# cerbos/cerbos

Measured on AMD Instinct MI355X. Metric: CheckResources decisions/sec at batch=1M; p50 per-decision us, higher is better.
Workload: dtype u32 ids + f64 attributes (CEL int64/uint64/double)

## Files before the change

cerbos_amd/csrc/cbh_check_flat.h:

```cpp
#pragma once
#include "cbh_check_wave.h"

#define CBH_FLAT_MAX_DEPTH 16
#if defined(CBH_FLAT_WAVES_OVERRIDE)
#define CBH_FLAT_WAVES CBH_FLAT_WAVES_OVERRIDE
#elif !defined(CBH_HOSTSIM)
#define CBH_FLAT_WAVES 4u
#else
#define CBH_FLAT_WAVES 1u
#endif
#define CBH_FLAT_THREADS (CBH_FLAT_WAVES * CBH_BLOCK)

__device__ __forceinline__ u64 wave_or64(u64 v, u32 wave, u32 lane) {
  __shared__ unsigned long long acc[CBH_FLAT_WAVES];
#ifndef CBH_HOSTSIM
  if (lane == 0) __hip_atomic_store(&acc[wave], 0ull, __ATOMIC_RELAXED, __HIP_MEMORY_SCOPE_WORKGROUP);
  (void)wave_ballot(true);
  if (v) (void)__hip_atomic_fetch_or(&acc[wave], (unsigned long long)v, __ATOMIC_RELAXED, __HIP_MEMORY_SCOPE_WORKGROUP);
  (void)wave_ballot(true);
  const u64 r = __hip_atomic_load(&acc[wave], __ATOMIC_RELAXED, __HIP_MEMORY_SCOPE_WORKGROUP);
#else
  if (lane == 0) acc[wave] = 0;
  (void)wave_ballot(true);
  if (v) atomicOr(&acc[wave], (unsigned long long)v);
  (void)wave_ballot(true);
  const u64 r = acc[wave];
#endif
  (void)wave_ballot(true);
  return r;
}

#define CBH_FLAT_LDS_STRINGS 4096u
struct u32x4u { u32 x, y, z, w; };
__device__ __forceinline__ u32x4u load_u32x4(const CBH_G u32* p) {
#ifndef CBH_HOSTSIM
  typedef u32 v4 __attribute__((ext_vector_type(4), aligned(4)));
  const v4 v = *(const CBH_G v4*)p;
  return u32x4u{v.x, v.y, v.z, v.w};
#else
  return u32x4u{p[0], p[1], p[2], p[3]};
#endif
}
template <int NDW> struct StagedRec { u32 w[NDW]; };
template <int NDW>
__device__ __forceinline__ StagedRec<NDW> stage_rec(const CBH_G u32* base, u32 idx, bool wanted) {
  StagedRec<NDW> r;
#pragma unroll
  for (int k = 0; k < NDW; ++k) r.w[k] = 0;
  if (wanted) {
    const CBH_G u32* p = base + (size_t)idx * NDW;
#pragma unroll
    for (int k = 0; k < NDW; k += 4) { const u32x4u v = load_u32x4(p + k); r.w[k] = v.x; r.w[k + 1] = v.y; r.w[k + 2] = v.z; r.w[k + 3] = v.w; }
  }
  return r;
}
template <typename R, int NDW>
__device__ __forceinline__ R staged_take(const StagedRec<NDW>& s, u32 lane) {
  static_assert(sizeof(R) == NDW * 4, "record size");
  u32 w[NDW];
#pragma unroll
  for (int k = 0; k < NDW; ++k) w[k] = wave_readlane(s.w[k], lane);
  R r;
  __builtin_memcpy(&r, w, sizeof(R));
  return r;
}
__device__ __forceinline__ u32 ctz64(u64 v) { return (u32)__builtin_ctzll(v); }
__device__ __forceinline__ u32 nz01(u32 v) {
#ifndef CBH_HOSTSIM
  u32 r;
  asm("v_min_u32 %0, 1, %1" : "=v"(r) : "v"(v));
  return r;
#else
  return v ? 1u : 0u;
#endif
}

template <typename T>
__device__ __forceinline__ void store_nt(CBH_G T* p, T v) {
#ifndef CBH_HOSTSIM
  __builtin_nontemporal_store(v, p);
#else
  *p = v;
#endif
}

struct __attribute__((aligned(64))) TblDrx { u32 rm_lo, rm_hi, flags, cond, name, p0, p1, p2; LeafRec leaf; };

struct FlatCol { u32 t, lo, hi; };
template <bool PT = false>
__device__ __forceinline__ FlatCol flat_col(const Ctx& c, u32 col, u32 req) {
  FlatCol v;
  v.t = cached_tag<PT>(c, col, req);
  v.lo = c.cc[col * CBH_BLOCK + c.tid];
  v.hi = c.cc[(c.n_cached + col) * CBH_BLOCK + c.tid];
  return v;
}
template <bool LISTS = true, bool PT = false>
__device__ __forceinline__ u32 flat_leaf(const Ctx& c, const LeafRec& lr, u32 req, u32 pid) {
  const u32 a = lr.w >> 8;
  const u32 ka = (a >> 8) & 0xFu, op = a & 0xFFu;
  const bool want_eq = op == OP_EQ;
  switch (lr.pad) {
    case 1: {
      const FlatCol x = flat_col<PT>(c, lr.a0, req);
      const bool err = x.t >= CBH_T_ABSENT;
      const bool eq = x.t == lr.ctag && x.lo == lr.clo;
      return err ? 2u : (u32)(eq == want_eq);
    }
    case 2: {
      const FlatCol x = flat_col<PT>(c, lr.a0, req);
      const bool err = x.t >= CBH_T_ABSENT;
      const bool dbl = x.t == CBH_T_DOUBLE, othernum = x.t == CBH_T_INT || x.t == CBH_T_UINT;
      const double p = as_f64((u64)x.lo | ((u64)x.hi << 32)), q = as_f64((u64)lr.clo | ((u64)lr.chi << 32));
      const bool ordering = op != OP_EQ && op != OP_NE;
      const bool cmp = (op == OP_EQ) ? p == q : (op == OP_NE) ? p != q : (op == OP_LT) ? p < q : (op == OP_LE) ? p <= q
                     : (op == OP_GT) ? p > q : p >= q;
      const bool slow = !err && othernum;
      const bool overload = !dbl && !othernum && ordering;
      const u32 r = dbl ? (u32)cmp : (u32)(op == OP_NE);
      return (err || overload) ? 2u : slow ? 4u : r;
    }
    case 3: {
      const FlatCol x = flat_col<PT>(c, lr.a0, req), y = flat_col<PT>(c, lr.a1, req);
      const bool err = x.t >= CBH_T_ABSENT || y.t >= CBH_T_ABSENT;
      const bool same = x.t == y.t;
      const bool scalar = x.t < CBH_T_LIST || x.t == CBH_T_TIMESTAMP || x.t == CBH_T_DURATION;
      const bool xnum = x.t == CBH_T_INT || x.t == CBH_T_UINT || x.t == CBH_T_DOUBLE, ynum = y.t == CBH_T_INT || y.t == CBH_T_UINT || y.t == CBH_T_DOUBLE;
      const bool bits_eq = x.lo == y.lo && x.hi == y.hi;
      const bool dbl_eq = as_f64((u64)x.lo | ((u64)x.hi << 32)) == as_f64((u64)y.lo | ((u64)y.hi << 32));
      const bool eq = same && (x.t == CBH_T_DOUBLE ? dbl_eq : bits_eq);
      const bool slow = !err && ((same && !scalar) || (!same && xnum && ynum));
      return err ? 2u : slow ? 4u : (u32)(eq == want_eq);
    }
    case 4: {
      const FlatCol x = flat_col<PT>(c, ka == 3 ? lr.a0 : lr.a1, req);
      const bool err = x.t >= CBH_T_ABSENT;
      const bool eq = x.t == CBH_T_STRING && x.lo == pid;
      return err ? 2u : (u32)(eq == want_eq);
    }
    case 6: {
      const FlatCol x = flat_col<PT>(c, lr.a0, req);
      const bool err = x.t >= CBH_T_ABSENT;
      const bool found = x.t == CBH_T_STRING && (x.lo == lr.ctag || x.lo == lr.clo || x.lo == lr.chi);
      return err ? 2u : (u32)found;
    }
    case 7:
    case 8: {
      if (!LISTS) return 4u;
      const FlatCol h = flat_col<PT>(c, lr.a1, req);
      u32 nt = CBH_T_STRING, nlo = lr.clo;
      bool err = h.t >= CBH_T_ABSENT;
      if (lr.pad == 8u) {
        if (ka == 4u) nlo = pid;
        else { const FlatCol x = flat_col<PT>(c, lr.a0, req); nt = x.t; nlo = x.lo; err = err || x.t >= CBH_T_ABSENT; }
      }
      const bool is_map = h.t == CBH_T_MAP, cont = h.t == CBH_T_LIST || is_map;
      const u32 sel = h.hi >> 30, off = h.hi & 0x3FFFFFFFu, len = cont ? h.lo : 0u, stride = is_map ? 2u : 1u;
      const bool slow = !err && (nt != CBH_T_STRING || (cont && (sel != CBH_HEAP_BATCH || len > 64u)));
      const u32 n = (err || slow) ? 0u : len;
      bool found = false;
      for (u32 i = 0; wave_ballot(i < n) != 0; i += 4u) {
        u32 tg[4]; u32 vl[4];
#pragma unroll
        for (u32 q = 0; q < 4; ++q) {
          const u32 at = off + stride * (i + q < n ? i + q : (n ? n - 1u : 0u));
          tg[q] = n ? (u32)c.b.heap_tag[at] : 0u; vl[q] = n ? (u32)c.b.heap_val[at] : 0u;
        }
#pragma unroll
        for (u32 q = 0; q < 4; ++q) found = found || (i + q < n && tg[q] == CBH_T_STRING && vl[q] == nlo);
      }
      return (err || (!slow && !cont)) ? 2u : slow ? 4u : (u32)found;
    }
    default: return 4u;
  }
}

template <bool LISTS = true, bool PT = false>
__device__ __forceinline__ u32 flat_tree(const Ctx& c, const LeafRec& desc, u32 req, u32 pid) {
  const u32 opw[4] = {desc.w, desc.a0, desc.ret, desc.ctag};
  bool live = true, last = false;
  u32 saved = 0, acc = 0, depth = 0, leaf = desc.a1, err = 0, slow = 0;
  for (u32 k = 0; k < 32; ++k) {
    const u32 ws = k >> 3, word = ws == 0u ? opw[0] : ws == 1u ? opw[1] : ws == 2u ? opw[2] : opw[3];
    const u32 op = (word >> (4u * (k & 7u))) & 15u;
    if (op == 0) break;
    if (op == 1) {
      const LeafRec lr = uload_rec<LeafRec>(c.t.code, leaf++);
      const u32 lv = flat_leaf<LISTS, PT>(c, lr, req, pid);
      last = live && (lv & 1u) != 0;
      err |= live ? (lv & 2u) : 0u;
      slow |= live ? (lv & 4u) : 0u;
    } else if (op < 5) {
      const u32 bit = 1u << depth;
      saved = live ? (saved | bit) : (saved & ~bit);
      acc = (op == 2) ? (acc | bit) : (acc & ~bit);
      ++depth;
    } else if (op < 8) {
      const u32 bit = 1u << (depth - 1u);
      const bool decides = live && ((op == 5) ? !last : last);
      acc = decides ? ((op == 5) ? (acc & ~bit) : (acc | bit)) : acc;
      live = live && !decides;
    } else {
      --depth;
      const u32 bit = 1u << depth;
      live = (saved & bit) != 0;
      last = ((acc & bit) != 0) != (op == 10);
    }
  }
  return slow ? 4u : ((u32)last | err);
}

__device__ __forceinline__ u32 wave_max_bits(u32 v, bool in, u32 nbits) {
  u32 best = 0;
  for (u32 k = nbits; k-- > 0;) {
    const bool bit = ((v >> k) & 1u) != 0;
    if (wave_ballot(in && bit) != 0) { in = in && bit; best |= 1u << k; }
  }
  return best;
}

#define CBH_LV_ROWS 16u
__device__ __forceinline__ u32 lv_code(const CBH_L u8* lvtab, u32 tid, u32 leaf) {
  return ((u32)lvtab[(leaf >> 2) * CBH_BLOCK + tid] >> ((leaf & 3u) * 2u)) & 3u;
}
__device__ __forceinline__ u32 lv_of_code(u32 code) { return code == 3u ? 4u : code; }
struct __attribute__((aligned(64))) Leaf4x4 { u32 w[16]; };
template <bool PT>
__device__ __forceinline__ void leaf_col(const Ctx& c, u32 w, u32 req, u32& curcol, FlatCol& x) {
  const u32 col = (w >> 16) & 0xFFu;
  if (col != curcol) { x = flat_col<PT>(c, col, req); curcol = col; }
}
template <bool PT>
__device__ __forceinline__ u32 leaf_block_codes(const Ctx& c, const Leaf4x4& b, u32 req, u32 pid, u32& curcol, FlatCol& x) {
  const u32 cls = b.w[0] & 15u;
  u32 acc = 0;
  if (cls == 1u) {
#pragma unroll
    for (u32 q = 0; q < 4; ++q) {
      const u32 w = b.w[4 * q];
      leaf_col<PT>(c, w, req, curcol, x);
      const bool ne = ((w >> 4) & 0xFFu) != OP_EQ;
      const bool eq = x.t == b.w[4 * q + 1] && x.lo == b.w[4 * q + 2];
      acc |= (x.t >= CBH_T_ABSENT ? 2u : (u32)(eq != ne)) << (2u * q);
    }
  } else if (cls == 2u) {
#pragma unroll
    for (u32 q = 0; q < 4; ++q) {
      const u32 w = b.w[4 * q], op = (w >> 4) & 0xFFu;
      leaf_col<PT>(c, w, req, curcol, x);
      const bool a_lt = op == OP_LT || op == OP_LE || op == OP_NE, a_eq = op == OP_EQ || op == OP_LE || op == OP_GE,
                 a_gt = op == OP_GT || op == OP_GE || op == OP_NE, a_un = op == OP_NE;
      const double p = as_f64((u64)x.lo | ((u64)x.hi << 32)), k = as_f64((u64)b.w[4 * q + 1] | ((u64)b.w[4 * q + 2] << 32));
      const bool lt = p < k, eq = p == k, gt = p > k;
      const bool cmp = (a_lt && lt) || (a_eq && eq) || (a_gt && gt) || (a_un && !(lt || eq || gt));
      const bool dbl = x.t == CBH_T_DOUBLE, othernum = x.t == CBH_T_INT || x.t == CBH_T_UINT;
      const bool ordering = op != OP_EQ && op != OP_NE;
      const u32 r = dbl ? (u32)cmp : (u32)(op == OP_NE);
// ... 207 lines not shown
    act_off = 4u * req;
  } else {
#define RQ(f) b.req_u32[(size_t)(f) * NR + req]
  pid = RQ(CBH_RQ_PRINCIPAL_ID); kind = RQ(CBH_RQ_KIND); r_scope = RQ(CBH_RQ_R_SCOPE); r_ver = RQ(CBH_RQ_R_VERSION);
  role_off = RQ(CBH_RQ_ROLE_OFF); act_off = RQ(CBH_RQ_ACT_OFF);
  role_cnt = valid ? RQ(CBH_RQ_ROLE_CNT) : 0; act_cnt = valid ? RQ(CBH_RQ_ACT_CNT) : 0;
#undef RQ
  if constexpr (AGROUP) {
    act_total = act_cnt;
    const u32 g4 = 4u * ag.group, left = act_cnt > g4 ? act_cnt - g4 : 0u;
    act_cnt = left < 4u ? left : 4u; act_off += g4;
  }
  if constexpr (!AGROUP) {
  spec = b.n_tuples >= 4u;
  spec_ix = (4u * req + 4u <= b.n_tuples) ? 4u * req : 0u;
  sp = load_u32x4(spec ? b.tuple_action + spec_ix : b.req_u32);
  }
  const u32 cls_i = threadIdx.x < t.K ? threadIdx.x : kmax;
  cls_a0 = (t.K ? t.action_class : (const CBH_G u8*)b.req_u32)[cls_i]; cls_r0 = (t.K ? t.role_class : (const CBH_G u8*)b.req_u32)[cls_i];
  }
  CcTags cct;
  if constexpr (COMPACT) { for (u32 g = 0; g < CBH_CACHE_COLS / 4; ++g) cct.w[g] = 0; } else cct = cc_load_tags(c, b, NR, w0, wd);
  const bool ptags = COMPACT || (c.flags & CBH_FI_PACKED_TAGS) != 0;
  const u32 all = CROSS ? ((1u << act_cnt) - 1u) & ~x_done : (1u << act_cnt) - 1u;
  const u32 max_depth = t.max_depth < CBH_FLAT_MAX_DEPTH ? t.max_depth : CBH_FLAT_MAX_DEPTH;
  const bool chain8 = t.n_scopes <= 256u;
  const u32 chain_dwords = chain8 ? max_depth * (CBH_BLOCK / 4u) : max_depth * CBH_BLOCK;
  CBH_L u32* chain_si = (CBH_L u32*)cbh_dyn_lds + CBH_FLAT_WAVES * CBH_CC_DWORDS(c.n_cached, ptags) + wave * chain_dwords;
  CBH_L u8* chain_si8 = (CBH_L u8*)chain_si;
  const bool cls_in_lds = t.K <= CBH_FLAT_LDS_STRINGS;
  CBH_L u8* cls_lds = (CBH_L u8*)((CBH_L u32*)cbh_dyn_lds + CBH_FLAT_WAVES * (CBH_CC_DWORDS(c.n_cached, ptags) + chain_dwords));
  u32 aid[4] = {0, 0, 0, 0}, rid[4] = {0, 0, 0, 0};
  if constexpr (!COMPACT) {
#pragma unroll
  for (u32 k = 0; k < 4; ++k) rid[k] = b.roles[k < role_cnt ? role_off + k : 0u];
  const bool spec_hit = spec && act_cnt == 4u && act_off == spec_ix;
  aid[0] = sp.x; aid[1] = sp.y; aid[2] = sp.z; aid[3] = sp.w;
  if (!spec_hit) {
#pragma unroll
    for (u32 k = 0; k < 4; ++k) aid[k] = b.tuple_action[k < act_cnt ? act_off + k : 0u];
  }
  if (cls_in_lds) {
    if (threadIdx.x < t.K) { cls_lds[threadIdx.x] = (u8)cls_a0; cls_lds[t.K + threadIdx.x] = (u8)cls_r0; }
    for (u32 i = threadIdx.x + CBH_FLAT_THREADS; i < t.K; i += CBH_FLAT_THREADS) { cls_lds[i] = t.action_class[i]; cls_lds[t.K + i] = t.role_class[i]; }
  }
  }
  CBH_L u64* segm = (CBH_L u64*)(cls_lds + (cls_in_lds ? ((2u * t.K + 15u) & ~15u) : 0u)) + wave * (CBH_SEG_LDS_BYTES / 8u);
  CBH_L u8* seg_rec = (CBH_L u8*)(segm + 64);
  CBH_L u64* seg_desc = segm + 64 + 16;
  CBH_L u8* lvtab = (CBH_L u8*)(segm + 64 + 16 + 64);
  CBH_L u32* ep_lds = (CBH_L u32*)(cls_lds + (cls_in_lds ? ((2u * t.K + 15u) & ~15u) : 0u) + (MODE == 2 ? CBH_FLAT_WAVES * CBH_SEG_LDS_BYTES : 0u)) + wave * max_depth * 2u * CBH_BLOCK;
  const bool want_ep = EP && (flags & CBH_F_WANT_EFFECTIVE_POLICIES) != 0 && o.eff_pol != nullptr;
  if (EP) { for (u32 d = 0; d < 2u * max_depth; ++d) ep_lds[d * CBH_BLOCK + c.tid] = 0; }
  if constexpr (CROSS) cc_fill_cross(c, b, NR, x_prow, x_rrow, x.side); else if constexpr (!COMPACT) cc_fill(c, b, NR, w0, wd, cct);
  const bool lenient = (flags & CBH_F_LENIENT_SCOPE_SEARCH) != 0;
  u32 first_own;
  if constexpr (COMPACT) first_own = c_first; else first_own = chain_first(t, r_scope, FLAG_RES, lenient);
  const u32 first = (AGROUP && ag.group != 0u && act_cnt == 0u) ? CBH_NONE : first_own;
  if constexpr (COMPACT) {
  } else if (cls_in_lds) {
    __syncthreads();
#pragma unroll
    for (u32 k = 0; k < 4; ++k) {
      const u32 ca = cls_lds[aid[k] < t.K ? aid[k] : kmax], cr = cls_lds[t.K + (rid[k] < t.K ? rid[k] : kmax)];
      ac[k] = (k < act_cnt && aid[k] < t.K && ca < 31u) ? ca : 31u;
      rc[k] = (k < role_cnt && rid[k] < t.K && cr < 31u) ? cr : 31u;
    }
  } else {
#pragma unroll
    for (u32 k = 0; k < 4; ++k) {
      const u32 ca = t.action_class[aid[k] < t.K ? aid[k] : kmax], cr = t.role_class[rid[k] < t.K ? rid[k] : kmax];
      ac[k] = (k < act_cnt && aid[k] < t.K && ca < 31u) ? ca : 31u;
      rc[k] = (k < role_cnt && rid[k] < t.K && cr < 31u) ? cr : 31u;
    }
  }
  u32 lane_ac = 0, lane_rc = 0;
  u32 walks = 0;
#pragma unroll
  for (u32 k = 0; k < 4; ++k) {
    if (k < act_cnt) lane_ac |= 1u << ac[k];
    if (k < role_cnt) { lane_rc |= 1u << rc[k]; walks |= all << (4 * k); }
  }
  const u64 wave_cls = wave_or64((u64)lane_ac | ((u64)lane_rc << 32), wave, c.tid);
  const u32 wave_ac = (u32)wave_cls, wave_rc = (u32)(wave_cls >> 32);
  FLAT_DBG(const u64 cyc1 = __builtin_readcyclecounter();)

  Lane L; L.req = req; L.edr = 0; L.status = 0; L.edr_err = false; L.pid = pid;

  u32 S = walks;
  u32 has_allow = 0, allow = 0, deny = 0, err = 0, unsup = 0;
  u32 dp0 = 0, dp1 = 0, dp2 = 0, dp3 = 0;
  const u32 scope_bits = t.n_scopes > 1 ? 32u - (u32)__builtin_clz(t.n_scopes - 1u) : 0u;

  auto leafish = [&](u32 ref, u32 how, const LeafRec& lr, bool active) -> u32 {
    u32 lv = 4u;
    FLAT_DBG(const u64 e0 = __builtin_readcyclecounter(); ++dbg_evals;)
    if (how == 1u) lv = flat_leaf<WITH_CALL || CROSS, COMPACT>(c, lr, req, pid);
    else if (how == 2u) lv = flat_tree<WITH_CALL || CROSS, COMPACT>(c, lr, req, pid);
    FLAT_DBG(cyc_eval += (__builtin_readcyclecounter() - e0) * (u64)(wave_ballot(lv != 77u) != 0);)
    const bool slow = active && lv == 4u;
    if (WITH_CALL) {
      if (wave_ballot(slow) != 0) {
        const u32 r = eval_ref<false>(c.ka_mem, lds_of(c), req, 0, false, ref, slow);
        if (slow) lv = ((r & 0xFFu) == 1u ? 1u : 0u) | (((r >> 8) & CBH_ST_CEL_ERROR) ? 2u : 0u) | (((r >> 8) & CBH_ST_UNSUPPORTED) ? 8u : 0u);
      }
    } else if (slow) lv = 8u;
    return active ? lv : 0u;
  };

  u32 memo_r0 = CBH_NONE, memo_r1 = CBH_NONE, memo_r2 = CBH_NONE, memo_r3 = CBH_NONE, memo_n = 0;
  u32 memo_lv = 0;
  auto leafish_memo = [&](u32 ref, u32 how, auto&& leaf, bool active) -> u32 {
    if constexpr (WITH_CALL || !MEMO) return leafish(ref, how, leaf(), active);
    else {
      const u32 j = ref == memo_r0 ? 0u : ref == memo_r1 ? 1u : ref == memo_r2 ? 2u : ref == memo_r3 ? 3u : 4u;
      if (j < 4u) return active ? ((memo_lv >> (4u * j)) & 15u) : 0u;
      const u32 lv = leafish(ref, how, leaf(), true);
      if (memo_n < 4u) {
        memo_r0 = memo_n == 0u ? ref : memo_r0; memo_r1 = memo_n == 1u ? ref : memo_r1; memo_r2 = memo_n == 2u ? ref : memo_r2; memo_r3 = memo_n == 3u ? ref : memo_r3;
        memo_lv |= lv << (4u * memo_n);
        ++memo_n;
      }
      return active ? lv : 0u;
    }
  };

  u32 cur = first, mydepth = 0;
  bool exists = false;
  const bool pooled = MODE == 2 && (t.seg_info & CBH_MSEG_POOLED) != 0;
  u32 blocks_done = 0;
  FLAT_DBG(const u64 cyc2 = cyc1 + (__builtin_readcyclecounter() - cyc1) * (u64)(wave_ballot(first != 0xFFFFFFFEu) != 0);)
  for (;;) {
    const bool active = cur != CBH_NONE && (S != 0 || !exists);
    if (wave_ballot(active) == 0) break;
    const u32 g_si = wave_max_bits(cur, active, scope_bits);
    const u64 here = wave_ballot(active && cur == g_si);
    const u32 lead = first_lane(here);
    const u32 g_ver = wave_readlane(r_ver, lead), g_k = wave_readlane(kind, lead);
    const bool ing = active && cur == g_si && r_ver == g_ver && kind == g_k;
    const bool go = wave_ballot(ing && S != 0) != 0;
    FLAT_DBG(++dbg_rounds;)
    uint4 bucket; bucket.x = bucket.y = bucket.z = bucket.w = 0;
    const bool have_bucket = udir_find(t, BTYPE, g_ver, g_k, g_si, bucket);
    exists = exists || (ing && have_bucket);
    if (go) {
      if (ing && mydepth < max_depth) { if (chain8) chain_si8[mydepth * CBH_BLOCK + c.tid] = (u8)g_si; else chain_si[mydepth * CBH_BLOCK + c.tid] = g_si; }
      const u32 S_before = S;
      u32 touch = 0, g_pol = 0;
      if constexpr (MODE == 2) {
        u32 blk16 = bucket.x;
        const bool any_seg = have_bucket && bucket.y != 0;
        SegHdr hd_nx = uload_rec<SegHdr>(t.segs, any_seg ? blk16 : 0u);
        const CBH_G u32* bn = t.segs + (size_t)(any_seg ? blk16 : 0u) * 16u;
        u64 m_nx = load_u64g(bn + 16u + 2u * c.tid), d_nx = load_u64g(bn + CBH_SEG_FIXED_DWORDS + 2u * c.tid);
        u32 r_nx = bn[144u + (c.tid & 31u)];
        for (u32 sgi = 0; any_seg && sgi < bucket.y && wave_ballot(ing && S != 0) != 0; ++sgi) {
          const CBH_G u32* blk = t.segs + (size_t)blk16 * 16u;
          const SegHdr hd = hd_nx;
          blk16 += hd.size16;
          if (!pooled) blocks_done = 0;
          segm[c.tid] = m_nx;
          if (c.tid < 32u) ((CBH_L u32*)seg_rec)[c.tid] = r_nx;
          seg_desc[c.tid] = d_nx;
          {
            const u32 nb16 = (sgi + 1u < bucket.y) ? blk16 : bucket.x;
            hd_nx = uload_rec<SegHdr>(t.segs, nb16);
            bn = t.segs + (size_t)nb16 * 16u;
            m_nx = load_u64g(bn + 16u + 2u * c.tid); d_nx = load_u64g(bn + CBH_SEG_FIXED_DWORDS + 2u * c.tid);
            r_nx = bn[144u + (c.tid & 31u)];
          }
          (void)wave_ballot(true);
          u64 A = 0, R = 0;
#pragma unroll
          for (u32 k = 0; k < 4; ++k) { if (k < act_cnt) A |= segm[ac[k]]; if (k < role_cnt) R |= segm[32u + rc[k]]; }
          const u64 cand_any = (ing && S != 0) ? (A & R) : 0ull;
          if (EP) {
            if (sgi == 0) g_pol = uload(&t.rows[(size_t)hd.row_begin * 16u + 3u]);
            if (cand_any != 0) {
#pragma unroll
              for (u32 k = 0; k < 4; ++k)
#pragma unroll
                for (u32 r = 0; r < 4; ++r)
                  if (((S >> (4u * r + k)) & 1u) && (segm[ac[k]] & segm[32u + rc[r]]) != 0) touch |= 1u << (4u * r + k);
            }
          }
          FLAT_DBG(dbg_rows += hd.n_records;)
          if (wave_ballot(cand_any != 0) != 0) {
            u64 csat = ~0ull, dsat = ~0ull, cerr = 0, derr = 0, cuns = 0, duns = 0;
            const u64 simple_c = (u64)hd.sc_lo | ((u64)hd.sc_hi << 32), simple_d = (u64)hd.sd_lo | ((u64)hd.sd_hi << 32);
            FLAT_DBG(const u64 i0 = __builtin_readcyclecounter();)
            const bool any_cond = hd.n_complex != 0 || wave_ballot((cand_any & (simple_c | simple_d)) != 0) != 0;
            if (any_cond) {
              const u32 nblk = ((pooled ? (t.seg_info & 0xFFu) : hd.n_leaves) + 3u) >> 2;
              const u32 todo = ~blocks_done & ((1u << nblk) - 1u);
              if (todo) {
                FLAT_DBG(const u64 l0 = __builtin_readcyclecounter();)
                eval_leaf_blocks<COMPACT>(c, pooled ? t.leafpool : blk + hd.off_leaves, todo, req, pid, lvtab);
                blocks_done |= todo;
                (void)wave_ballot(true);
                FLAT_DBG(cyc_stage += (__builtin_readcyclecounter() - l0) * (u64)(wave_ballot(req != 0xdeadbeefu) != 0); dbg_visits += (u32)__builtin_popcount(todo);)
              }
            }
            for (u32 ci = 0; ci < hd.n_complex; ++ci) {
              const SegItem it = uload_rec<SegItem>(blk + (hd.off_rc >> 16), ci);
              const u64 cc = (u64)it.cc_lo | ((u64)it.cc_hi << 32), cd = (u64)it.cd_lo | ((u64)it.cd_hi << 32);
              const bool need = ((cc | cd) & cand_any) != 0;
              if (wave_ballot(need) == 0) continue;
              FLAT_DBG(++dbg_evals;)
              const u64 idx = (u64)it.idx_lo | ((u64)it.idx_hi << 32);
              u32 lv = 4u;
              if ((it.how & 3u) == 1u) {
                u32 w = 0;
                for (u32 j = 0; j < it.n_leaves; ++j) w |= lv_code(lvtab, c.tid, (u32)(idx >> (8u * j)) & 0xFFu) << (2u * j);
                lv = level_from_codes(w, it.n_leaves, (it.how & 256u) != 0, (it.how & 512u) != 0);
              } else if ((it.how & 3u) == 2u) lv = tree_from_codes(it.ops, idx, lvtab, c.tid);
              const bool slow = need && lv == 4u;
              if (WITH_CALL) {
                if (wave_ballot(slow) != 0) {
                  const u32 r = eval_ref<false>(c.ka_mem, lds_of(c), req, 0, false, it.ref, slow);
                  if (slow) lv = ((r & 0xFFu) == 1u ? 1u : 0u) | (((r >> 8) & CBH_ST_CEL_ERROR) ? 2u : 0u) | (((r >> 8) & CBH_ST_UNSUPPORTED) ? 8u : 0u);
                }
              } else if (slow) lv = 8u;
              csat &= (lv & 1u) ? ~0ull : ~cc; dsat &= (lv & 1u) ? ~0ull : ~cd;
              cerr |= (lv & 2u) ? cc : 0ull; derr |= (lv & 2u) ? cd : 0ull; cuns |= (lv & 8u) ? cc : 0ull; duns |= (lv & 8u) ? cd : 0ull;
            }
            u64 cslow = 0, dslow = 0;
            u32 lane_slow = 0;
            auto lane_items = [&](u64 m, const CBH_L u8* rec, u64& sat, u64& errm, u64& slowm) {
              while (wave_ballot(m != 0) != 0) {
                const bool act = m != 0;
                const u32 i = act ? ctz64(m) : 0u;
// ... 27 lines not shown
                  const bool is_d = lc == 0;
                  const u32 i = ctz64(is_d ? ldd : lc);
                  const u64 bit = 1ull << i;
                  const u32 itx = uniform((u32)seg_rec[(is_d ? CBH_SEG_RECORDS : 0u) + i]);
                  const u32 ref = uload(blk + (hd.off_rc & 0xFFFFu) + itx);
                  const bool mine = ((is_d ? dslow : cslow) & bit) != 0;
                  const u32 r = eval_ref<false>(c.ka_mem, lds_of(c), req, 0, false, ref, mine);
                  if (mine) {
                    const bool ok = (r & 0xFFu) == 1u, e = ((r >> 8) & CBH_ST_CEL_ERROR) != 0, u = ((r >> 8) & CBH_ST_UNSUPPORTED) != 0;
                    if (is_d) { dslow &= ~bit; dsat = ok ? (dsat | bit) : dsat; derr |= e ? bit : 0ull; duns |= u ? bit : 0ull; }
                    else { cslow &= ~bit; csat = ok ? (csat | bit) : csat; cerr |= e ? bit : 0ull; cuns |= u ? bit : 0ull; }
                  }
                }
              }
            }
            if (!WITH_CALL && lane_slow) { cuns |= cand_any; duns |= cand_any; }
            FLAT_DBG(cyc_eval += (__builtin_readcyclecounter() - i0) * (u64)(wave_ballot(csat != 77u) != 0);)
            const u64 satrec = dsat & csat, errrec = derr | (dsat & cerr), unsrec = duns | (dsat & cuns);
            const u64 allow_m = (u64)hd.allow_lo | ((u64)hd.allow_hi << 32), deny_m = (u64)hd.deny_lo | ((u64)hd.deny_hi << 32);
            const bool anybad = wave_ballot(((errrec | unsrec) & cand_any) != 0) != 0;
            const u32 live16 = ing ? S : 0u;
            if (anybad) {
              const u64 badc = cand_any & (errrec | unsrec);
#pragma unroll
              for (u32 r = 0; r < 4; ++r) {
                const u64 rmk = segm[32u + rc[r]];
                const bool rlive = ((live16 >> (4u * r)) & 0xFu) != 0;
                if (wave_ballot(rlive && (rmk & badc) != 0) == 0) continue;
#pragma unroll
                for (u32 k = 0; k < 4; ++k) {
                  const u32 bit = 1u << (4u * r + k);
                  const u64 cand = (live16 & bit) ? (rmk & segm[ac[k]]) : 0ull;
                  if (wave_ballot((cand & badc) != 0) == 0) continue;
                  const u64 dh = cand & satrec & deny_m;
                  const u64 below = dh ? (((dh & (0ull - dh)) << 1) - 1ull) : ~0ull;
                  err |= (cand & errrec & below) ? bit : 0u;
                  unsup |= (cand & unsrec & below) ? bit : 0u;
                }
              }
            }
            u32 a_lo[4], a_hi[4], d_lo[4], d_hi[4];
#pragma unroll
            for (u32 k = 0; k < 4; ++k) {
              const u64 am = segm[ac[k]] & satrec;
              a_lo[k] = (u32)(am & allow_m); a_hi[k] = (u32)((am & allow_m) >> 32);
              d_lo[k] = (u32)(am & deny_m); d_hi[k] = (u32)((am & deny_m) >> 32);
            }
            u32 A16 = 0, D16 = 0;
#pragma unroll
            for (u32 rr = 0; rr < 4; ++rr) {
              const u32 r = 3u - rr;
              if (wave_ballot(((live16 >> (4u * r)) & 0xFu) != 0) == 0) { A16 <<= 4; D16 <<= 4; continue; }
              const u64 rmk = segm[32u + rc[r]];
              const u32 r_lo = (u32)rmk, r_hi = (u32)(rmk >> 32);
#pragma unroll
              for (u32 kk = 0; kk < 4; ++kk) {
                const u32 k = 3u - kk;
                const u32 ta = (r_hi & a_hi[k]) | (r_lo & a_lo[k]), td = (r_hi & d_hi[k]) | (r_lo & d_lo[k]);
                A16 = (A16 << 1) | nz01(ta);
                D16 = (D16 << 1) | nz01(td);
              }
            }
            A16 &= live16; D16 &= live16;
            has_allow |= A16;
            deny |= D16; S &= ~D16;
          }
          (void)wave_ballot(true);
        }
      } else if constexpr (STAGED) {
        if (have_bucket && bucket.y) {
          const u32 end = bucket.x + bucket.y;
          for (u32 base = bucket.x; base < end && wave_ballot(ing && S != 0) != 0; base += CBH_BLOCK) {
            const u32 n = end - base < CBH_BLOCK ? end - base : CBH_BLOCK;
            const bool mine = c.tid < n;
            FLAT_DBG(const u64 g0 = __builtin_readcyclecounter();)
            const StagedRec<16> sr = stage_rec<16>(t.rows, base + c.tid, mine);
            const StagedRec<8> s2 = stage_rec<8>(t.rowleaf2, base + c.tid, mine && sr.w[2] != CBH_NONE);
            u64 cand = wave_ballot(mine && (sr.w[4] & wave_rc) != 0 && (sr.w[6] & wave_ac) != 0);
            FLAT_DBG(dbg_rows += n; cyc_stage += (__builtin_readcyclecounter() - g0) * (u64)(cand != 0xdeadbeefull);)
            while (cand != 0) {
              const u32 i = ctz64(cand);
              cand &= cand - 1ull;
              const u32 row = base + i;
              const TblRowFull rf = staged_take<TblRowFull>(sr, i);
              const TblRow& rw = rf.hot;
              const u32 mact = ((rw.am_lo >> ac[0]) & 1u) | (((rw.am_lo >> ac[1]) & 1u) << 1) | (((rw.am_lo >> ac[2]) & 1u) << 2) | (((rw.am_lo >> ac[3]) & 1u) << 3);
              const u32 mrole = ((0u - ((rw.rm_lo >> rc[0]) & 1u)) & 0xFu) | ((0u - ((rw.rm_lo >> rc[1]) & 1u)) & 0xF0u) |
                                ((0u - ((rw.rm_lo >> rc[2]) & 1u)) & 0xF00u) | ((0u - ((rw.rm_lo >> rc[3]) & 1u)) & 0xF000u);
              const u32 m = ing ? (mrole & (mact * 0x1111u) & S) : 0u;
              if (wave_ballot(m != 0) == 0) continue;
              if (EP) touch |= m;
              FLAT_DBG(++dbg_visits;)
              u32 hit = m;
              if (rw.drcond != CBH_NONE) {
                const u32 how = (rw.flags & CBH_ROW_F_DRLEAF_EMBEDDED) ? 1u : (rw.flags & CBH_ROW_F_DRTREE_EMBEDDED) ? 2u : 0u;
                const u32 lv = leafish_memo(rw.drcond, how, [&] { return staged_take<LeafRec>(s2, i); }, hit != 0);
                err |= (lv & 2u) ? hit : 0u; unsup |= (lv & 8u) ? hit : 0u;
                hit = (lv & 1u) ? hit : 0u;
              }
              if (rw.cond != CBH_NONE && wave_ballot(hit != 0) != 0) {
                const u32 how = (rw.flags & CBH_ROW_F_LEAF_EMBEDDED) ? 1u : (rw.flags & CBH_ROW_F_TREE_EMBEDDED) ? 2u : 0u;
                const u32 lv = leafish(rw.cond, how, rf.leaf, hit != 0);
                err |= (lv & 2u) ? hit : 0u; unsup |= (lv & 8u) ? hit : 0u;
                hit = (lv & 1u) ? hit : 0u;
              }
              if ((rw.flags & 3u) == CBH_EFFECT_ALLOW) has_allow |= hit;
              else if ((rw.flags & 3u) == CBH_EFFECT_DENY) { deny |= hit; S &= ~hit; }
              (void)row;
            }
          }
        }
      } else {
        if (have_bucket && bucket.y) {
          const u32 last = bucket.x + bucket.y - 1u;
          TblRowFull nxt = uload_rec<TblRowFull>(t.rows, bucket.x);
          for (u32 row = bucket.x; row <= last; ++row) {
            const TblRowFull rf = nxt;
            nxt = uload_rec<TblRowFull>(t.rows, row < last ? row + 1u : last);
            const TblRow& rw = rf.hot;
            FLAT_DBG(++dbg_rows;)
            if ((rw.rm_lo & wave_rc) == 0 || (rw.am_lo & wave_ac) == 0) continue;
            const u32 mact = ((rw.am_lo >> ac[0]) & 1u) | (((rw.am_lo >> ac[1]) & 1u) << 1) | (((rw.am_lo >> ac[2]) & 1u) << 2) | (((rw.am_lo >> ac[3]) & 1u) << 3);
            const u32 mrole = ((0u - ((rw.rm_lo >> rc[0]) & 1u)) & 0xFu) | ((0u - ((rw.rm_lo >> rc[1]) & 1u)) & 0xF0u) |
                              ((0u - ((rw.rm_lo >> rc[2]) & 1u)) & 0xF00u) | ((0u - ((rw.rm_lo >> rc[3]) & 1u)) & 0xF000u);
            const u32 m = ing ? (mrole & (mact * 0x1111u) & S) : 0u;
            if (wave_ballot(m != 0) == 0) continue;
            if (EP) touch |= m;
            u32 hit = m;
            if (rw.drcond != CBH_NONE) {
              const u32 how = (rw.flags & CBH_ROW_F_DRLEAF_EMBEDDED) ? 1u : (rw.flags & CBH_ROW_F_DRTREE_EMBEDDED) ? 2u : 0u;
              const u32 lv = leafish_memo(rw.drcond, how, [&] { return uload_rec<LeafRec>(t.rowleaf2, row); }, hit != 0);
              err |= (lv & 2u) ? hit : 0u; unsup |= (lv & 8u) ? hit : 0u;
              hit = (lv & 1u) ? hit : 0u;
            }
            if (rw.cond != CBH_NONE && wave_ballot(hit != 0) != 0) {
              const u32 how = (rw.flags & CBH_ROW_F_LEAF_EMBEDDED) ? 1u : (rw.flags & CBH_ROW_F_TREE_EMBEDDED) ? 2u : 0u;
              const u32 lv = leafish(rw.cond, how, rf.leaf, hit != 0);
              err |= (lv & 2u) ? hit : 0u; unsup |= (lv & 8u) ? hit : 0u;
              hit = (lv & 1u) ? hit : 0u;
            }
            if ((rw.flags & 3u) == CBH_EFFECT_ALLOW) has_allow |= hit;
            else if ((rw.flags & 3u) == CBH_EFFECT_DENY) { deny |= hit; S &= ~hit; }
          }
        }
      }
      if (EP) {
        if (MODE != 2 && have_bucket && bucket.y) g_pol = uload(&t.rows[(size_t)bucket.x * 16u + 3u]);
        if (ing && mydepth < max_depth) { ep_lds[(2u * mydepth) * CBH_BLOCK + c.tid] = touch; ep_lds[(2u * mydepth + 1u) * CBH_BLOCK + c.tid] = g_pol; }
      }
      const u32 ha = ing ? (has_allow & S) : 0u;
      const u32 sp = (uload(&t.scope_flags[g_si]) >> 2) & 3u;
      if (sp == SP_REQUIRE_CONSENT) has_allow &= ~ha;
      else if (sp == SP_OVERRIDE_PARENT) { allow |= ha; S &= ~ha; }
      if (max_depth > 1u) {
        const u32 newly = S_before & ~S;
        dp0 |= (mydepth & 1u) ? newly : 0u; dp1 |= (mydepth & 2u) ? newly : 0u; dp2 |= (mydepth & 4u) ? newly : 0u; dp3 |= (mydepth & 8u) ? newly : 0u;
      }
    }
    const u32 up = (COMPACT && max_depth <= 1u) ? CBH_NONE : uchain_next(t, uload(&t.scope_parent[g_si]), FLAG_RES);
    if (ing) { cur = (mydepth + 1u < max_depth) ? up : CBH_NONE; ++mydepth; }
  }

  FLAT_DBG(const u64 cyc3 = __builtin_readcyclecounter();)
  const bool decided = first == CBH_NONE || !exists;
  const u32 pol_none = (u32)(decided ? CBH_P_NO_MATCH : (role_cnt ? CBH_P_RESOURCE : CBH_P_EMPTY)) << 28 | ((!decided && role_cnt) ? first : 0u);
  const u32 pol_hit = ((u32)CBH_P_RESOURCE << 28) | first;
  const u32 st_ok = (t.flags & CBH_MF_TRACE_ALL) ? CBH_ST_WANTS_TRACE : CBH_ST_OK;
  bool alw[4], won[4];
  u32 sc1[4];
#pragma unroll
  for (u32 k = 0; k < 4; ++k) {
    const u32 ak = allow & (0x1111u << k), dk = deny & (0x1111u << k);
    const u32 sel = ak ? ak : dk;
    const u32 wb = sel & (0u - sel);
    alw[k] = ak != 0; won[k] = sel != 0;
    u32 s = first;
    if (max_depth > 1u) {
      const u32 d = ((dp0 & wb) ? 1u : 0u) | ((dp1 & wb) ? 2u : 0u) | ((dp2 & wb) ? 4u : 0u) | ((dp3 & wb) ? 8u : 0u);
      s = chain8 ? (u32)chain_si8[d * CBH_BLOCK + c.tid] : chain_si[d * CBH_BLOCK + c.tid];
    }
    sc1[k] = (won[k] && k < act_cnt) ? s + 1u : 0u;
  }
  u32 st4 = st_ok * 0x01010101u;
  if (wave_ballot((err | unsup) != 0) != 0) {
    st4 = 0;
#pragma unroll
    for (u32 k = 0; k < 4; ++k) {
      const u32 ak = (allow >> k) & 0x1111u;
      const u32 seen = ak ? (((ak & (0u - ak)) << 1) - 1u) : 0xFFFFu;
      const u32 ek = (err >> k) & 0x1111u & seen, uk = (unsup >> k) & 0x1111u & seen;
      st4 |= (u32)(uk ? CBH_ST_UNSUPPORTED : (ek ? CBH_ST_CEL_ERROR : st_ok)) << (8 * k);
    }
  }

  if (EP && want_ep && valid) {
    u32 legit = 0;
#pragma unroll
    for (u32 k = 0; k < 4; ++k) {
      const u32 ak = (allow >> k) & 0x1111u;
      const u32 seen = ak ? (((ak & (0u - ak)) << 1) - 1u) : 0xFFFFu;
      legit |= ((walks >> k) & 0x1111u & seen) << k;
    }
    for (u32 d = 0; d < max_depth; ++d)
      if (ep_lds[(2u * d) * CBH_BLOCK + c.tid] & legit) ep_mark(o, b, req, ep_lds[(2u * d + 1u) * CBH_BLOCK + c.tid]);
  }
  u64 edr = 0;
  if ((flags & CBH_F_WANT_DERIVED_ROLES) && t.n_dr) {
    u32 legit = 0;
#pragma unroll
    for (u32 k = 0; k < 4; ++k) {
      const u32 ak = (allow >> k) & 0x1111u;
      const u32 seen = ak ? (((ak & (0u - ak)) << 1) - 1u) : 0xFFFFu;
      legit |= ((walks >> k) & 0x1111u & seen) << k;
    }
    const u32 done = allow | deny;
    u32 reach = 0;
    if (legit & ~done) reach = CBH_FLAT_MAX_DEPTH;
    else if (legit) {
      u32 cand = legit, d = 0;
      u32 tp = cand & dp3; if (tp) { cand = tp; d |= 8u; }
      tp = cand & dp2; if (tp) { cand = tp; d |= 4u; }
      tp = cand & dp1; if (tp) { cand = tp; d |= 2u; }
      tp = cand & dp0; if (tp) { cand = tp; d |= 1u; }
      reach = d + 1u;
    }
// ... 398 lines not shown
```

Measured before the change: 188.0 billion.

## Unify row visit path, use bitfield-extract matching, and double-buffer row loads

```diff
diff --git a/cerbos_amd/csrc/cbh_check_flat.h b/cerbos_amd/csrc/cbh_check_flat.h
--- a/cerbos_amd/csrc/cbh_check_flat.h
+++ b/cerbos_amd/csrc/cbh_check_flat.h
@@ -64,6 +64,32 @@
   __builtin_memcpy(&r, w, sizeof(R));
   return r;
 }
+__device__ __forceinline__ u32 bit_at(u32 word, u32 pos) {
+#ifndef CBH_HOSTSIM
+  return __builtin_amdgcn_ubfe(word, pos, 1u);
+#else
+  return (word >> (pos & 31u)) & 1u;
+#endif
+}
+__device__ __forceinline__ u32 flat_match(u32 rm_lo, u32 am_lo, const u32 (&ac)[4], const u32 (&rc)[4]) {
+  const u32 mact = bit_at(am_lo, ac[0]) | (bit_at(am_lo, ac[1]) << 1) | (bit_at(am_lo, ac[2]) << 2) | (bit_at(am_lo, ac[3]) << 3);
+  const u32 mrole = bit_at(rm_lo, rc[0]) | (bit_at(rm_lo, rc[1]) << 4) | (bit_at(rm_lo, rc[2]) << 8) | (bit_at(rm_lo, rc[3]) << 12);
+  return mrole * mact;
+}
+__device__ __forceinline__ u32 index_behind(u32 idx, u32 arrived) {
+#ifndef CBH_HOSTSIM
+  asm volatile("" : "+s"(idx) : "s"(arrived));
+#else
+  (void)arrived;
+#endif
+  return idx;
+}
+#ifdef CBH_HOSTSIM
+inline unsigned long long cbh_sim_record_steps = 0, cbh_sim_record_visits = 0;
+#define CBH_SIM_COUNT(x) do { if (c.tid == 0) ++(x); } while (0)
+#else
+#define CBH_SIM_COUNT(x)
+#endif
 __device__ __forceinline__ u32 ctz64(u64 v) { return (u32)__builtin_ctzll(v); }
 __device__ __forceinline__ u32 nz01(u32 v) {
 #ifndef CBH_HOSTSIM
@@ -95,84 +121,84 @@
   v.hi = c.cc[(c.n_cached + col) * CBH_BLOCK + c.tid];
   return v;
 }
-template <bool LISTS = true, bool PT = false>
-__device__ __forceinline__ u32 flat_leaf(const Ctx& c, const LeafRec& lr, u32 req, u32 pid) {
+template <bool LISTS = true, bool PT = false, typename OUT>
+__device__ __forceinline__ auto flat_leaf_to(const Ctx& c, const LeafRec& lr, u32 req, u32 pid, OUT&& out) {
   const u32 a = lr.w >> 8;
   const u32 ka = (a >> 8) & 0xFu, op = a & 0xFFu;
   const bool want_eq = op == OP_EQ;
-  switch (lr.pad) {
-    case 1: {
-      const FlatCol x = flat_col<PT>(c, lr.a0, req);
-      const bool err = x.t >= CBH_T_ABSENT;
-      const bool eq = x.t == lr.ctag && x.lo == lr.clo;
-      return err ? 2u : (u32)(eq == want_eq);
-    }
-    case 2: {
-      const FlatCol x = flat_col<PT>(c, lr.a0, req);
-      const bool err = x.t >= CBH_T_ABSENT;
-      const bool dbl = x.t == CBH_T_DOUBLE, othernum = x.t == CBH_T_INT || x.t == CBH_T_UINT;
-      const double p = as_f64((u64)x.lo | ((u64)x.hi << 32)), q = as_f64((u64)lr.clo | ((u64)lr.chi << 32));
-      const bool ordering = op != OP_EQ && op != OP_NE;
-      const bool cmp = (op == OP_EQ) ? p == q : (op == OP_NE) ? p != q : (op == OP_LT) ? p < q : (op == OP_LE) ? p <= q
-                     : (op == OP_GT) ? p > q : p >= q;
-      const bool slow = !err && othernum;
-      const bool overload = !dbl && !othernum && ordering;
-      const u32 r = dbl ? (u32)cmp : (u32)(op == OP_NE);
-      return (err || overload) ? 2u : slow ? 4u : r;
-    }
-    case 3: {
-      const FlatCol x = flat_col<PT>(c, lr.a0, req), y = flat_col<PT>(c, lr.a1, req);
-      const bool err = x.t >= CBH_T_ABSENT || y.t >= CBH_T_ABSENT;
-      const bool same = x.t == y.t;
-      const bool scalar = x.t < CBH_T_LIST || x.t == CBH_T_TIMESTAMP || x.t == CBH_T_DURATION;
-      const bool xnum = x.t == CBH_T_INT || x.t == CBH_T_UINT || x.t == CBH_T_DOUBLE, ynum = y.t == CBH_T_INT || y.t == CBH_T_UINT || y.t == CBH_T_DOUBLE;
-      const bool bits_eq = x.lo == y.lo && x.hi == y.hi;
-      const bool dbl_eq = as_f64((u64)x.lo | ((u64)x.hi << 32)) == as_f64((u64)y.lo | ((u64)y.hi << 32));
-      const bool eq = same && (x.t == CBH_T_DOUBLE ? dbl_eq : bits_eq);
-      const bool slow = !err && ((same && !scalar) || (!same && xnum && ynum));
-      return err ? 2u : slow ? 4u : (u32)(eq == want_eq);
-    }
-    case 4: {
-      const FlatCol x = flat_col<PT>(c, ka == 3 ? lr.a0 : lr.a1, req);
-      const bool err = x.t >= CBH_T_ABSENT;
-      const bool eq = x.t == CBH_T_STRING && x.lo == pid;
-      return err ? 2u : (u32)(eq == want_eq);
-    }
-    case 6: {
-      const FlatCol x = flat_col<PT>(c, lr.a0, req);
-      const bool err = x.t >= CBH_T_ABSENT;
-      const bool found = x.t == CBH_T_STRING && (x.lo == lr.ctag || x.lo == lr.clo || x.lo == lr.chi);
-      return err ? 2u : (u32)found;
-    }
-    case 7:
-    case 8: {
-      if (!LISTS) return 4u;
-      const FlatCol h = flat_col<PT>(c, lr.a1, req);
-      u32 nt = CBH_T_STRING, nlo = lr.clo;
-      bool err = h.t >= CBH_T_ABSENT;
-      if (lr.pad == 8u) {
-        if (ka == 4u) nlo = pid;
-        else { const FlatCol x = flat_col<PT>(c, lr.a0, req); nt = x.t; nlo = x.lo; err = err || x.t >= CBH_T_ABSENT; }
+  const u32 cls = lr.pad;
+  if (uniform(cls) == 1u) {
+    const FlatCol x = flat_col<PT>(c, lr.a0, req);
+    const bool err = x.t >= CBH_T_ABSENT;
+    const bool eq = x.t == lr.ctag && x.lo == lr.clo;
+    return out(err, eq == want_eq, false);
+  }
+  if (cls == 4u) {
+    const FlatCol x = flat_col<PT>(c, ka == 3 ? lr.a0 : lr.a1, req);
+    const bool err = x.t >= CBH_T_ABSENT;
+    const bool eq = x.t == CBH_T_STRING && x.lo == pid;
+    return out(err, eq == want_eq, false);
+  }
+  if (cls == 2u) {
+    const FlatCol x = flat_col<PT>(c, lr.a0, req);
+    const bool err = x.t >= CBH_T_ABSENT;
+    const bool dbl = x.t == CBH_T_DOUBLE, othernum = x.t == CBH_T_INT || x.t == CBH_T_UINT;
+    const double p = as_f64((u64)x.lo | ((u64)x.hi << 32)), q = as_f64((u64)lr.clo | ((u64)lr.chi << 32));
+    const bool ordering = op != OP_EQ && op != OP_NE;
+    const bool cmp = (op == OP_EQ) ? p == q : (op == OP_NE) ? p != q : (op == OP_LT) ? p < q : (op == OP_LE) ? p <= q
+                   : (op == OP_GT) ? p > q : p >= q;
+    const bool slow = !err && othernum;
+    const bool overload = !dbl && !othernum && ordering;
+    return out(err || overload, dbl ? cmp : op == OP_NE, slow);
+  }
+  if (cls == 3u) {
+    const FlatCol x = flat_col<PT>(c, lr.a0, req), y = flat_col<PT>(c, lr.a1, req);
+    const bool err = x.t >= CBH_T_ABSENT || y.t >= CBH_T_ABSENT;
+    const bool same = x.t == y.t;
+    const bool scalar = x.t < CBH_T_LIST || x.t == CBH_T_TIMESTAMP || x.t == CBH_T_DURATION;
+    const bool xnum = x.t == CBH_T_INT || x.t == CBH_T_UINT || x.t == CBH_T_DOUBLE, ynum = y.t == CBH_T_INT || y.t == CBH_T_UINT || y.t == CBH_T_DOUBLE;
+    const bool bits_eq = x.lo == y.lo && x.hi == y.hi;
+    const bool dbl_eq = as_f64((u64)x.lo | ((u64)x.hi << 32)) == as_f64((u64)y.lo | ((u64)y.hi << 32));
+    const bool eq = same && (x.t == CBH_T_DOUBLE ? dbl_eq : bits_eq);
+    const bool slow = !err && ((same && !scalar) || (!same && xnum && ynum));
+    return out(err, eq == want_eq, slow);
+  }
+  if (cls == 6u) {
+    const FlatCol x = flat_col<PT>(c, lr.a0, req);
+    const bool err = x.t >= CBH_T_ABSENT;
+    const bool found = x.t == CBH_T_STRING && (x.lo == lr.ctag || x.lo == lr.clo || x.lo == lr.chi);
+    return out(err, found, false);
+  }
+  if (LISTS && (cls == 7u || cls == 8u)) {
+    const FlatCol h = flat_col<PT>(c, lr.a1, req);
+    u32 nt = CBH_T_STRING, nlo = lr.clo;
+    bool err = h.t >= CBH_T_ABSENT;
+    if (cls == 8u) {
+      if (ka == 4u) nlo = pid;
+      else { const FlatCol x = flat_col<PT>(c, lr.a0, req); nt = x.t; nlo = x.lo; err = err || x.t >= CBH_T_ABSENT; }
+    }
+    const bool is_map = h.t == CBH_T_MAP, cont = h.t == CBH_T_LIST || is_map;
+    const u32 sel = h.hi >> 30, off = h.hi & 0x3FFFFFFFu, len = cont ? h.lo : 0u, stride = is_map ? 2u : 1u;
+    const bool slow = !err && (nt != CBH_T_STRING || (cont && (sel != CBH_HEAP_BATCH || len > 64u)));
+    const u32 n = (err || slow) ? 0u : len;
+    bool found = false;
+    for (u32 i = 0; wave_ballot(i < n) != 0; i += 4u) {
+      u32 tg[4]; u32 vl[4];
+#pragma unroll
+      for (u32 q = 0; q < 4; ++q) {
+        const u32 at = off + stride * (i + q < n ? i + q : (n ? n - 1u : 0u));
+        tg[q] = n ? (u32)c.b.heap_tag[at] : 0u; vl[q] = n ? (u32)c.b.heap_val[at] : 0u;
       }
-      const bool is_map = h.t == CBH_T_MAP, cont = h.t == CBH_T_LIST || is_map;
-      const u32 sel = h.hi >> 30, off = h.hi & 0x3FFFFFFFu, len = cont ? h.lo : 0u, stride = is_map ? 2u : 1u;
-      const bool slow = !err && (nt != CBH_T_STRING || (cont && (sel != CBH_HEAP_BATCH || len > 64u)));
-      const u32 n = (err || slow) ? 0u : len;
-      bool found = false;
-      for (u32 i = 0; wave_ballot(i < n) != 0; i += 4u) {
-        u32 tg[4]; u32 vl[4];
-#pragma unroll
-        for (u32 q = 0; q < 4; ++q) {
-          const u32 at = off + stride * (i + q < n ? i + q : (n ? n - 1u : 0u));
-          tg[q] = n ? (u32)c.b.heap_tag[at] : 0u; vl[q] = n ? (u32)c.b.heap_val[at] : 0u;
-        }
-#pragma unroll
-        for (u32 q = 0; q < 4; ++q) found = found || (i + q < n && tg[q] == CBH_T_STRING && vl[q] == nlo);
-      }
-      return (err || (!slow && !cont)) ? 2u : slow ? 4u : (u32)found;
-    }
-    default: return 4u;
-  }
+#pragma unroll
+      for (u32 q = 0; q < 4; ++q) found = found || (i + q < n && tg[q] == CBH_T_STRING && vl[q] == nlo);
+    }
+    return out(err || (!slow && !cont), found, slow);
+  }
+  return out(false, false, true);
+}
+template <bool LISTS = true, bool PT = false>
+__device__ __forceinline__ u32 flat_leaf(const Ctx& c, const LeafRec& lr, u32 req, u32 pid) {
+  return flat_leaf_to<LISTS, PT>(c, lr, req, pid, [](bool err, bool sat, bool slow) -> u32 { return err ? 2u : slow ? 4u : (u32)sat; });
 }
 
 template <bool LISTS = true, bool PT = false>
@@ -546,7 +572,7 @@
     if (k < role_cnt) { lane_rc |= 1u << rc[k]; walks |= all << (4 * k); }
   }
   const u64 wave_cls = wave_or64((u64)lane_ac | ((u64)lane_rc << 32), wave, c.tid);
-  const u32 wave_ac = (u32)wave_cls, wave_rc = (u32)(wave_cls >> 32);
+  const u32 wave_ac = MEMO ? uniform((u32)wave_cls) : (u32)wave_cls, wave_rc = MEMO ? uniform((u32)(wave_cls >> 32)) : (u32)(wave_cls >> 32);
   FLAT_DBG(const u64 cyc1 = __builtin_readcyclecounter();)
 
   Lane L; L.req = req; L.edr = 0; L.status = 0; L.edr_err = false; L.pid = pid;
@@ -587,6 +613,35 @@
       }
       return active ? lv : 0u;
     }
+  };
+
+  auto apply_lv = [&](u32 lv, u32& hit) {
+    err |= (lv & 2u) ? hit : 0u; unsup |= (lv & 8u) ? hit : 0u;
+    hit = (lv & 1u) ? hit : 0u;
+  };
+  auto leaf_on = [&](const LeafRec& lr, u32& hit) {
+    FLAT_DBG(const u64 e0 = __builtin_readcyclecounter(); ++dbg_evals;)
+    flat_leaf_to<CROSS, COMPACT>(c, lr, req, pid, [&](bool e, bool sat, bool slow) -> u32 {
+      err |= e ? hit : 0u;
+      unsup |= (!e && slow) ? hit : 0u;
+      hit = (!e && !slow && sat) ? hit : 0u;
+      return 0u;
+    });
+    FLAT_DBG(cyc_eval += (__builtin_readcyclecounter() - e0) * (u64)(wave_ballot(hit != 77u) != 0);)
+  };
+  auto own_cond = [&](const TblRow& rw, const LeafRec& leaf, u32& hit) {
+    if constexpr (!WITH_CALL) {
+      if (rw.flags & CBH_ROW_F_LEAF_EMBEDDED) { leaf_on(leaf, hit); return; }
+    }
+    const u32 how = (rw.flags & CBH_ROW_F_LEAF_EMBEDDED) ? 1u : (rw.flags & CBH_ROW_F_TREE_EMBEDDED) ? 2u : 0u;
+    apply_lv(leafish(rw.cond, how, leaf, hit != 0), hit);
+  };
+  auto dr_cond = [&](const TblRow& rw, auto&& leaf, u32& hit) {
+    if constexpr (!WITH_CALL && !MEMO) {
+      if (rw.flags & CBH_ROW_F_DRLEAF_EMBEDDED) { leaf_on(leaf(), hit); return; }
+    }
+    const u32 how = (rw.flags & CBH_ROW_F_DRLEAF_EMBEDDED) ? 1u : (rw.flags & CBH_ROW_F_DRTREE_EMBEDDED) ? 2u : 0u;
+    apply_lv(leafish_memo(rw.drcond, how, leaf, hit != 0), hit);
   };
 
   u32 cur = first, mydepth = 0;
@@ -611,6 +666,24 @@
       if (ing && mydepth < max_depth) { if (chain8) chain_si8[mydepth * CBH_BLOCK + c.tid] = (u8)g_si; else chain_si[mydepth * CBH_BLOCK + c.tid] = g_si; }
       const u32 S_before = S;
       u32 touch = 0, g_pol = 0;
+      u32 S_in = ing ? S : 0u;
+      auto visit = [&](const TblRowFull& rf, auto&& drleaf) {
+        const TblRow& rw = rf.hot;
+        const u32 m = flat_match(rw.rm_lo, rw.am_lo, ac, rc) & S_in;
+        if (wave_ballot(m != 0) == 0) return;
+        if (EP) touch |= m;
+        FLAT_DBG(if (STAGED) ++dbg_visits;)
+        u32 hit = m;
+        if (rw.drcond != CBH_NONE) {
+          dr_cond(rw, drleaf, hit);
+          if (wave_ballot(hit != 0) == 0) return;
+        }
+        if (rw.cond != CBH_NONE) own_cond(rw, rf.leaf, hit);
+        const u32 eff = rw.flags & 3u;
+        if (uniform(eff) == CBH_EFFECT_ALLOW) has_allow |= hit;
+        else if (eff == CBH_EFFECT_DENY) { deny |= hit; S &= ~hit; S_in &= ~hit; }
+      };
+      (void)visit; (void)S_in;
       if constexpr (MODE == 2) {
         u32 blk16 = bucket.x;
         const bool any_seg = have_bucket && bucket.y != 0;
@@ -804,30 +877,7 @@
               const u32 i = ctz64(cand);
               cand &= cand - 1ull;
               const u32 row = base + i;
-              const TblRowFull rf = staged_take<TblRowFull>(sr, i);
-              const TblRow& rw = rf.hot;
-              const u32 mact = ((rw.am_lo >> ac[0]) & 1u) | (((rw.am_lo >> ac[1]) & 1u) << 1) | (((rw.am_lo >> ac[2]) & 1u) << 2) | (((rw.am_lo >> ac[3]) & 1u) << 3);
-              const u32 mrole = ((0u - ((rw.rm_lo >> rc[0]) & 1u)) & 0xFu) | ((0u - ((rw.rm_lo >> rc[1]) & 1u)) & 0xF0u) |
-                                ((0u - ((rw.rm_lo >> rc[2]) & 1u)) & 0xF00u) | ((0u - ((rw.rm_lo >> rc[3]) & 1u)) & 0xF000u);
-              const u32 m = ing ? (mrole & (mact * 0x1111u) & S) : 0u;
-              if (wave_ballot(m != 0) == 0) continue;
-              if (EP) touch |= m;
-              FLAT_DBG(++dbg_visits;)
-              u32 hit = m;
-              if (rw.drcond != CBH_NONE) {
-                const u32 how = (rw.flags & CBH_ROW_F_DRLEAF_EMBEDDED) ? 1u : (rw.flags & CBH_ROW_F_DRTREE_EMBEDDED) ? 2u : 0u;
-                const u32 lv = leafish_memo(rw.drcond, how, [&] { return staged_take<LeafRec>(s2, i); }, hit != 0);
-                err |= (lv & 2u) ? hit : 0u; unsup |= (lv & 8u) ? hit : 0u;
-                hit = (lv & 1u) ? hit : 0u;
-              }
-              if (rw.cond != CBH_NONE && wave_ballot(hit != 0) != 0) {
-                const u32 how = (rw.flags & CBH_ROW_F_LEAF_EMBEDDED) ? 1u : (rw.flags & CBH_ROW_F_TREE_EMBEDDED) ? 2u : 0u;
-                const u32 lv = leafish(rw.cond, how, rf.leaf, hit != 0);
-                err |= (lv & 2u) ? hit : 0u; unsup |= (lv & 8u) ? hit : 0u;
-                hit = (lv & 1u) ? hit : 0u;
-              }
-              if ((rw.flags & 3u) == CBH_EFFECT_ALLOW) has_allow |= hit;
-              else if ((rw.flags & 3u) == CBH_EFFECT_DENY) { deny |= hit; S &= ~hit; }
+              visit(staged_take<TblRowFull>(sr, i), [&] { return staged_take<LeafRec>(s2, i); });
               (void)row;
             }
           }
@@ -835,34 +885,28 @@
       } else {
         if (have_bucket && bucket.y) {
           const u32 last = bucket.x + bucket.y - 1u;
-          TblRowFull nxt = uload_rec<TblRowFull>(t.rows, bucket.x);
-          for (u32 row = bucket.x; row <= last; ++row) {
-            const TblRowFull rf = nxt;
-            nxt = uload_rec<TblRowFull>(t.rows, row < last ? row + 1u : last);
-            const TblRow& rw = rf.hot;
+          auto step = [&](const TblRowFull& rf, u32 row) {
             FLAT_DBG(++dbg_rows;)
-            if ((rw.rm_lo & wave_rc) == 0 || (rw.am_lo & wave_ac) == 0) continue;
-            const u32 mact = ((rw.am_lo >> ac[0]) & 1u) | (((rw.am_lo >> ac[1]) & 1u) << 1) | (((rw.am_lo >> ac[2]) & 1u) << 2) | (((rw.am_lo >> ac[3]) & 1u) << 3);
-            const u32 mrole = ((0u - ((rw.rm_lo >> rc[0]) & 1u)) & 0xFu) | ((0u - ((rw.rm_lo >> rc[1]) & 1u)) & 0xF0u) |
-                              ((0u - ((rw.rm_lo >> rc[2]) & 1u)) & 0xF00u) | ((0u - ((rw.rm_lo >> rc[3]) & 1u)) & 0xF000u);
-            const u32 m = ing ? (mrole & (mact * 0x1111u) & S) : 0u;
-            if (wave_ballot(m != 0) == 0) continue;
-            if (EP) touch |= m;
-            u32 hit = m;
-            if (rw.drcond != CBH_NONE) {
-              const u32 how = (rw.flags & CBH_ROW_F_DRLEAF_EMBEDDED) ? 1u : (rw.flags & CBH_ROW_F_DRTREE_EMBEDDED) ? 2u : 0u;
-              const u32 lv = leafish_memo(rw.drcond, how, [&] { return uload_rec<LeafRec>(t.rowleaf2, row); }, hit != 0);
-              err |= (lv & 2u) ? hit : 0u; unsup |= (lv & 8u) ? hit : 0u;
-              hit = (lv & 1u) ? hit : 0u;
-            }
-            if (rw.cond != CBH_NONE && wave_ballot(hit != 0) != 0) {
-              const u32 how = (rw.flags & CBH_ROW_F_LEAF_EMBEDDED) ? 1u : (rw.flags & CBH_ROW_F_TREE_EMBEDDED) ? 2u : 0u;
-              const u32 lv = leafish(rw.cond, how, rf.leaf, hit != 0);
-              err |= (lv & 2u) ? hit : 0u; unsup |= (lv & 8u) ? hit : 0u;
-              hit = (lv & 1u) ? hit : 0u;
-            }
-            if ((rw.flags & 3u) == CBH_EFFECT_ALLOW) has_allow |= hit;
-            else if ((rw.flags & 3u) == CBH_EFFECT_DENY) { deny |= hit; S &= ~hit; }
+            CBH_SIM_COUNT(cbh_sim_record_steps);
+            if ((rf.hot.rm_lo & wave_rc) == 0 || (rf.hot.am_lo & wave_ac) == 0) return;
+            CBH_SIM_COUNT(cbh_sim_record_visits);
+            visit(rf, [&] { return uload_rec<LeafRec>(t.rowleaf2, row); });
+          };
+          TblRowFull ra = uload_rec<TblRowFull>(t.rows, bucket.x);
+          if constexpr (MEMO) for (u32 row = bucket.x; row <= last; ++row) {
+            const TblRowFull rf = ra;
+            ra = uload_rec<TblRowFull>(t.rows, row < last ? row + 1u : last);
+            step(rf, row);
+          }
+          else for (u32 row = bucket.x;;) {
+            const TblRowFull rb = uload_rec<TblRowFull>(t.rows, index_behind(row < last ? row + 1u : last, ra.hot.rm_lo));
+            step(ra, row);
+            if (row == last) break;
+            ++row;
+            ra = uload_rec<TblRowFull>(t.rows, index_behind(row < last ? row + 1u : last, rb.hot.rm_lo));
+            step(rb, row);
+            if (row == last) break;
+            ++row;
           }
         }
       }
```

Result: no change. 187.0 billion (-0.6%).
